# PacificBiosciences/trgt

Hardware: AMD Instinct MI355X
Metric: loci/s (higher is better)
Workload: dtype u8/u16 (WFA) + f64 (HMM); 1 GPU; BASELINE configs[1]: 10000 synthetic single-motif STR loci per GPU (motif 3-6 bp, allele <= 200 bp), 30 reads/locus HiFi-like, 10% truncated reads (SURVEY.md Appendix E), seed 20250509; contexts_per_gpu=4, loci_per_gpu=10000, reads_per_locus=30, parallelism=loci sharded across 1 GPU(s), no collective

## Files before the change

trgt_amd/csrc/common.hpp:

```cpp
#pragma once
#include <hip/hip_runtime.h>

#include <cstdarg>
#include <cstdint>
#include <cstdio>
#include <cstring>
#include <ctime>
#include <algorithm>
#include <mutex>
#include <string>
#include <vector>

#include "../../include/trgt_hip.h"

#ifdef TRGT_DEV_BUILD
#define TRGT_DEV_ENV(name) getenv(name)
#else
#define TRGT_DEV_ENV(name) ((const char*)nullptr)
#endif

struct trgt_knobs {
  int filter_force = 0;
  int flank_threads = 256;
  int heavy_band = 96;
// ... 16 lines not shown
  bool no_indel_shortcut = false;
  bool no_hamming = false;
  bool no_filter = false;
  bool one_stream = false;
  bool host_genotyper = false;
  bool no_early = false;
  bool stage_lock = false;
  bool host_hmm_lists = false;
  bool debug = false;
  bool hmm_resolve_one_wg = false;
  bool wfa_no_wave_variant = false;
  bool wfa_no_stage = false;
  bool filter_side = false;
  bool filter_serial = false;
  bool filter_one_launch = false;
  bool no_long_window = false;
  bool no_long_filter = false;
  bool no_lean = false;
  bool lean_mid_tier = false;
  int lean_chunk = 0;
  bool no_zero_arena = false;
  bool hmm_ppl_per_class = false;
  bool hmm_ppl_wide = false;
  bool hmm_ppl_serial = false;
  bool lean_one_tier = false;
  bool no_lds_wfa = true;
  int lds_wfa_kb = 7;
  int lds_wfa_seq = 768;
  int sens_bialign_min_len = -1;
  bool sens_cons_unidir = false;
  bool sens_ward_ties = false;
  bool sens_lw_order = false;
  bool hmm_no_dedupe = false;
  bool hmm_no_long_tb = false;
  int hmm_long_wgs = 4;
  bool hmm_no_ppl = false;
  bool hmm_four_rounds = false;
  bool hmm_lds_fill = false;
  int cluster_arena_kb = 0;
  int repair_arena_kb = 0;
  bool host_cluster = false;
  bool host_purity = false;
  bool host_repair = false;
  bool split_hmm = false;
  int repair_blocks = 2048;
  int repair_max_seg = 0;
// ... 491 lines not shown
```

trgt_amd/csrc/ctx.hip:

```cpp
#include "common.hpp"
#include "host_pool.hpp"

static std::string g_create_err;

#include <malloc.h>
static void tune_malloc_once() {
  static std::once_flag once;
  std::call_once(once, [] {
    const char* e = getenv("TRGT_MALLOC_TUNE");
    const int mode = e && *e ? atoi(e) : 1;
    if (mode <= 0) return;
    (void)mallopt(M_MMAP_THRESHOLD, 32 << 20);
    (void)mallopt(M_TRIM_THRESHOLD, 1 << 30);
    (void)mallopt(M_TOP_PAD, 64 << 20);
    if (mode >= 2) (void)mallopt(M_MMAP_MAX, 0);
  });
}

namespace trgt {
static thread_local int g_next_stream_priority = 0;
static thread_local bool g_next_in_pool = false;
void ctx_next_stream_priority(int p) { g_next_stream_priority = p; }
void ctx_next_in_pool(bool on) { g_next_in_pool = on; }
hipError_t make_stream(trgt_hip_ctx* c, hipStream_t* s) {
// ... 34 lines not shown
    return TRGT_ERR_NO_DEVICE;
  }
  tune_malloc_once();
  trgt_hip_ctx* c = new trgt_hip_ctx();
  {
    trgt_knobs& k = c->knobs;
    auto num = [](const char* name, int dflt) { const char* e = getenv(name); return e && *e ? atoi(e) : dflt; };
    auto flag = [](const char* name) { const char* e = getenv(name); return e != nullptr && *e != 0 && std::strcmp(e, "0") != 0; };
#ifdef TRGT_DEV_BUILD
#define DEV_FLAG(name) flag(name)
#define DEV_NUM(name, dflt) num(name, dflt)
#else
#define DEV_FLAG(name) false
#define DEV_NUM(name, dflt) (dflt)
#endif
    (void)num; (void)flag;
    k.flank_threads = DEV_NUM("TRGT_FLANK_THREADS", k.flank_threads); k.heavy_threads = DEV_NUM("TRGT_HEAVY_THREADS", 0); k.heavy_band = std::max(0, std::min(num("TRGT_HEAVY_BAND", k.heavy_band), 256));
    k.win_threads = DEV_NUM("TRGT_WIN_THREADS", k.win_threads); { const int bt = DEV_NUM("TRGT_BAND_THREADS", k.band_threads); k.band_threads = bt == 128 || bt == 256 ? bt : 64; } k.win_segments = DEV_NUM("TRGT_WIN_SEGMENTS", k.win_segments); k.win_lds = DEV_FLAG("TRGT_WIN_LDS"); k.band_lds = DEV_FLAG("TRGT_BAND_LDS");
    k.grid_per_cu = DEV_NUM("TRGT_WFA_GRID_PER_CU", 0); k.filter_per_cu = DEV_NUM("TRGT_FILTER_PER_CU", 0);
    k.one_launch = DEV_FLAG("TRGT_WFA_ONE_LAUNCH"); k.no_spec = DEV_FLAG("TRGT_WFA_NO_SPEC"); k.no_window = flag("TRGT_WFA_NO_WINDOW"); k.no_hamming = flag("TRGT_NO_HAMMING"); k.no_indel_shortcut = flag("TRGT_NO_INDEL_SHORTCUT"); k.no_heavy_window = DEV_FLAG("TRGT_NO_HEAVY_WINDOW"); k.no_sibling_rule = DEV_FLAG("TRGT_NO_SIBLING_RULE"); k.no_settled_sibling_rule = DEV_FLAG("TRGT_NO_SETTLED_SIBLING_RULE"); k.no_lcs_rule = DEV_FLAG("TRGT_NO_LCS_RULE"); { const char* e = TRGT_DEV_ENV("TRGT_EARLY_ADAPTIVE"); if (e && *e) k.early_adaptive = std::strcmp(e, "0") != 0; }
    k.no_filter = flag("TRGT_WFA_NO_FILTER"); k.one_stream = DEV_FLAG("TRGT_FLANK_ONE_STREAM"); k.host_genotyper = flag("TRGT_HOST_GENOTYPER"); k.host_hmm_lists = DEV_FLAG("TRGT_HOST_HMM_LISTS"); k.no_early = flag("TRGT_WFA_NO_EARLY"); k.stage_lock = flag("TRGT_STAGE_LOCK"); k.no_long_filter = flag("TRGT_NO_LONG_FILTER"); k.no_long_window = DEV_FLAG("TRGT_NO_LONG_WINDOW"); k.filter_force = DEV_NUM("TRGT_FILTER_FORCE", 0); k.filter_one_launch = DEV_FLAG("TRGT_FILTER_ONE_LAUNCH"); k.filter_serial = DEV_FLAG("TRGT_FILTER_SERIAL"); k.filter_side = DEV_FLAG("TRGT_FILTER_SIDE"); k.wfa_no_stage = DEV_FLAG("TRGT_WFA_NO_STAGE"); k.wfa_no_wave_variant = DEV_FLAG("TRGT_WFA_NO_WAVE_VARIANT"); k.hmm_resolve_one_wg = DEV_FLAG("TRGT_HMM_RESOLVE_ONE_WG"); k.debug = flag("TRGT_WFA_DEBUG");
    k.timeline = flag("TRGT_TIMELINE");
    k.host_repair = flag("TRGT_HOST_REPAIR"); k.host_cluster = flag("TRGT_HOST_CLUSTER"); k.host_purity = DEV_FLAG("TRGT_HOST_PURITY"); k.cluster_arena_kb = num("TRGT_CLUSTER_ARENA_KB", 0); k.repair_arena_kb = num("TRGT_REPAIR_ARENA_KB", 0); k.hmm_lds_fill = DEV_FLAG("TRGT_HMM_LDS_FILL"); k.hmm_four_rounds = DEV_FLAG("TRGT_HMM_FOUR_ROUNDS"); k.hmm_no_ppl = flag("TRGT_HMM_NO_PPL"); k.hmm_long_wgs = std::max(1, std::min(DEV_NUM("TRGT_HMM_LONG_WGS", k.hmm_long_wgs), 16)); k.hmm_no_long_tb = flag("TRGT_HMM_NO_LONG_TB"); k.hmm_no_dedupe = flag("TRGT_HMM_NO_DEDUPE"); k.repair_max_seg = num("TRGT_REPAIR_MAX_SEG", k.repair_max_seg); k.split_hmm = DEV_FLAG("TRGT_SPLIT_HMM"); k.repair_blocks = DEV_NUM("TRGT_REPAIR_BLOCKS", k.repair_blocks);
    k.no_lean = flag("TRGT_WFA_NO_LEAN"); k.lean_one_tier = DEV_FLAG("TRGT_WFA_LEAN_ONE_TIER"); k.lean_mid_tier = DEV_FLAG("TRGT_WFA_LEAN_MID_TIER"); k.lean_chunk = DEV_NUM("TRGT_LEAN_CHUNK", 0); k.no_zero_arena = flag("TRGT_NO_ZERO_ARENA"); k.hmm_ppl_serial = DEV_FLAG("TRGT_HMM_PPL_SERIAL"); k.hmm_ppl_wide = DEV_FLAG("TRGT_HMM_PPL_WIDE"); k.hmm_ppl_per_class = DEV_FLAG("TRGT_HMM_PPL_PER_CLASS");
    k.no_lds_wfa = !DEV_FLAG("TRGT_WFA_LDS"); k.lds_wfa_kb = DEV_NUM("TRGT_WFA_LDS_KB", k.lds_wfa_kb); k.lds_wfa_seq = DEV_NUM("TRGT_WFA_LDS_SEQ", k.lds_wfa_seq);
#ifdef TRGT_DEV_BUILD
    k.sens_bialign_min_len = num("TRGT_SENS_BIALIGN_MIN_LEN", -1); k.sens_cons_unidir = flag("TRGT_SENS_CONS_UNIDIR"); k.sens_ward_ties = flag("TRGT_SENS_WARD_TIES"); k.sens_lw_order = flag("TRGT_SENS_LW_ORDER");
    k.skip_bt = flag("TRGT_DBG_SKIP_BT");
#endif
  }
  c->device = device;
  c->num_cus = prop.multiProcessorCount;
  c->stream_priority = trgt::g_next_stream_priority;
  c->in_pool = trgt::g_next_in_pool;
  e = trgt::make_stream(c, &c->stream);
  if (e != hipSuccess) { g_create_err = hipGetErrorString(e); delete c; return TRGT_ERR_HIP; }
  c->own_stream = true;
  c->pool.resize(trgt::S_COUNT);
  *out = c;
  return TRGT_OK;
}

void trgt_hip_destroy(trgt_hip_ctx* c) {
  if (!c) return;
  (void)hipSetDevice(c->device);
  (void)trgt::stream_wait(c, c->stream);
  if (c->stream2) { (void)trgt::stream_wait(c, c->stream2); (void)hipStreamDestroy(c->stream2); }
// ... 92 lines not shown
```

trgt_amd/csrc/hmm.hip:

```cpp
#include <algorithm>
#include <type_traits>
#include <cmath>
#include <limits>
#include <thread>

#include "common.hpp"

namespace trgt {


}
#include <memory>

#include "hmm_host.hpp"
namespace trgt {

struct HmmJobDev {
  uint32_t set, seq_len, job_index, path_cap;
  uint64_t seq_off, bp_off, path_off, span_off, count_off, visit_off;
  uint64_t map_off;
};

static inline uint64_t align_up(uint64_t v, uint64_t a) { return (v + a - 1) / a * a; }

// ... 433 lines not shown
  for (int i = tid; i < 4 * S; i += nthr) l_inst[4 * (i % S) + i / S] = hmm_pred_entry(g_inst[i], S, nb, model + set.off_flags, g_block, g_blocks);
  const bool own_fill = !(ppl_filled && set.ppl_lanes != 0u);
  for (int i = tid; i < S; i += nthr) { l_block[i] = g_block[i]; l_flags[i] = model[set.off_flags + i]; if (own_fill) { l_lp[i] = g_inlp[i]; l_lp[S + i] = g_inlp[S + i]; } }
  if (own_fill) for (int i = tid; i < 5 * S; i += nthr) l_em[i] = g_em[i];
  for (int i = tid; i < 4 * nb; i += nthr) l_blocks[i] = g_blocks[i];

  const int st_lane = set.n_lanes ? (int)reinterpret_cast<const uint16_t*>(model + set.off_perm)[tid] : tid;
  const bool act = st_lane < S;
  const int st = act ? st_lane : 0;
  const int n_in = own_fill ? (int)model[set.off_nin + st] : 0;
  const int level = own_fill ? (int)model[set.off_level + st] : 0;
  double lp0 = 0.0, lp1 = 0.0, lp2 = 0.0, lp3 = 0.0;
  int p0 = 0, p1 = 0, p2 = 0, p3 = 0;
  if (own_fill) {
    lp0 = g_inlp[0 * S + st]; lp1 = g_inlp[1 * S + st]; lp2 = g_inlp[2 * S + st]; lp3 = g_inlp[3 * S + st];
    p0 = g_inst[0 * S + st]; p1 = g_inst[1 * S + st]; p2 = g_inst[2 * S + st]; p3 = g_inst[3 * S + st];
  }
  const int q0 = (n_in != 0xFF && n_in > 0) ? p0 : 0, q1 = (n_in != 0xFF && n_in > 1) ? p1 : 0, q2 = (n_in != 0xFF && n_in > 2) ? p2 : 0, q3 = (n_in != 0xFF && n_in > 3) ? p3 : 0;
  const uint8_t* __restrict__ seq = seq_blob + job.seq_off;
  int win0 = 0;
  auto code_at = [&](int i) -> int { return (int)l_seq[i - win0]; };
  uint8_t* __restrict__ bp = bp_ws + job.bp_off;
  hmm_sync_mem(sync_n);
  if (act) {
    const int blk = (int)l_block[st];
    uint32_t kind = 0, expected = 0;
    if (blk >= 0) {
      const int bstart = (int)l_blocks[0 * nb + blk], bend = (int)l_blocks[1 * nb + blk];
      if (st == bstart) kind = 1;
      else if (st == bend) kind = 2;
      else if (blk == nb - 1) kind = 3;
      else {
        const int mlen = (int)l_blocks[2 * nb + blk], off = st - bstart - 1, k = off / mlen;
        kind = 4u + (uint32_t)k;
        if (k == 0) expected = motif_bytes[l_blocks[3 * nb + blk] + off];
      }
    }
    l_info[st] = kind | ((uint32_t)(l_flags[st] & 1) << 3) | ((uint32_t)(blk & 0xFF) << 8) | (expected << 16);
  }
  const int my_blk = act ? (int)l_block[st] : -1;
  const bool role_end = act && my_blk >= 0 && st == (int)l_blocks[1 * nb + my_blk];
  const bool role_start = act && my_blk >= 0 && st == (int)l_blocks[0 * nb + my_blk];
  const bool role_del = act && level > 0 && !role_end && !role_start && n_in != 0xFF && my_blk >= 0;
  const bool role_chain = role_del || role_end;
  const bool chain_prev = role_del ? n_in > 1 : role_end ? n_in > 2 : false;
  const bool chain_xwave = chain_prev && (threadIdx.x & 63u) == 0;
  const double lp_chain = role_del ? lp1 : lp2, lp_step = chain_prev && !chain_xwave ? lp_chain : NINF;
  const int chain_steps = __builtin_amdgcn_readfirstlane(min(63, max((int)set.max_mlen, SUB == 32 ? __shfl_xor((int)set.max_mlen, 32) : 0) - 1));
  const int chain_rounds = (int)set.chain_rounds;
  const bool wave_chain = __ballot(lp_step > NINF) != 0ull;

  HP_MARK(0);
  const double lp_rs0 = l_lp[1], lp_rs1 = l_lp[S + 1];
  constexpr int BE_REG = 8;
  int be[BE_REG];
#pragma unroll
  for (int b = 0; b < BE_REG; ++b) be[b] = (int)l_blocks[1 * nb + (b < nb ? b : 0)];
  const int my_ms = my_blk >= 0 ? (int)l_blocks[0 * nb + my_blk] : 0, my_me = my_blk >= 0 ? (int)l_blocks[1 * nb + my_blk] : 0;
  const double ms_lp0 = my_blk >= 0 ? l_lp[my_ms] : NINF, ms_lp1 = my_blk >= 0 ? l_lp[S + my_ms] : NINF;
  bool bad = false, use_loc0 = false, use_loc1 = false;
  if (own_fill && act && my_blk >= 0) bad = model[set.off_nin + my_ms] != 2 || g_inst[0 * S + my_ms] != 1 || g_inst[1 * S + my_ms] != my_me;
  if (own_fill && act && level == 0 && n_in != 0xFF) {
// ... 449 lines not shown
  hmm_sync_mem(sync_n);

  const bool packed = ppl_filled && ppl_packed && set.ppl_lanes != 0u;
  const int rstride = packed ? hmm_ppl_group(set.ppl_lanes) : Spad;
  const int cols_per_chunk = packed ? hmm_stage_bytes(Spad) / rstride - 2 : max(1, hmm_stage_bytes(Spad) / Spad);
  if (tid == 0) tb[TB_LOC] = 0;
  uint16_t* pbuf = path ? path + job.path_off : nullptr;
  uint32_t* const g_vis = visit_ws + job.visit_off;
  const int pcap = (int)job.path_cap;
  constexpr int HMM_REC = SUB == 32 ? 32 : 64;
  const unsigned long long gmask = SUB == 32 ? (0xFFFFFFFFull << (threadIdx.x & 32u)) : ~0ull;
  const HmmSyncN sync{sync_n};
  const HmmTraceLds tl{tb, l_inst, l_info, l_blocks, l_flags, l_stage, l_seq, l_mot, l_vis, l_cnt, l_rec};
  hmm_trace_rounds<HMM_REC, true>(sync, tid, nthr, tl, packed, rstride, cols_per_chunk, S, nb, L, seq, bp, g_vis, pbuf, pcap, gmask);
  const int np = tb[TB_NPATH];
  HP_MARK(2);
  hmm_path_to_front(sync, tid, nthr, pbuf, np, pcap);
  if (tid == 0) hmm_store_purity(job.job_index, np, tb[TB_EDIT], tb[TB_REF], qlen, path_len, purity, edit_out, maxd_out);
  hmm_decode_visits(sync, tid, nthr, tl, nb, g_vis, spans3 + 3 * job.span_off, n_spans + job.job_index, counts + job.count_off);
  HP_MARK(3);
}

#include "hmm_ppl.hpp"
#include "hmm_big.hpp"

struct HmmChunkMap { uint16_t exit_state, last_state, n_steps, n_starts; int32_t last_end; };
struct HmmChunkRec { uint32_t entry, np0, nv0; int32_t vb0, nxt0; uint32_t pad[3]; };
constexpr int HMM_LONG_THREADS = 1024, HMM_LONG_STG = 2048;
constexpr int HMM_LONG_MAP_LDS = 48 * 1024;

__global__ void __launch_bounds__(HMM_LONG_THREADS) hmm_traceback_long_kernel(
    const HmmJobDev* __restrict__ jobs, const HmmSetDev* __restrict__ sets, const uint8_t* __restrict__ model, const uint8_t* __restrict__ seq_blob,
    const uint8_t* __restrict__ bp_ws, uint32_t* __restrict__ visit_ws, uint16_t* __restrict__ path, uint32_t* __restrict__ path_len,
    int32_t* __restrict__ spans3, uint32_t* __restrict__ n_spans, uint32_t* __restrict__ counts, double* __restrict__ purity,
    int32_t* __restrict__ edit_out, int32_t* __restrict__ maxd_out, const uint32_t* __restrict__ long_list, const int phase_arg, const int G) {
  const int phase = phase_arg & 0xFF;
  const bool ppl_packed = ((phase_arg >> 8) & 1) != 0;
  extern __shared__ __align__(16) unsigned char lds_long[];
  const int tid = (int)threadIdx.x, lane = tid & 63, wave = tid >> 6;
  constexpr int NW = HMM_LONG_THREADS / 64;
  const int part = (int)(blockIdx.x % (unsigned)G);
  __shared__ int l_last;
  for (uint32_t li = blockIdx.x / (unsigned)G; li < long_list[0]; li += gridDim.x / (unsigned)G) {
    __syncthreads();
    const HmmJobDev job = jobs[long_list[1 + li]];
    const HmmSetDev set = sets[job.set];
// ... 499 lines not shown
```

trgt_amd/csrc/hmm_batch.hpp:

```cpp
#pragma once

static inline uint32_t hmm_long_min(uint64_t class_jobs) { return class_jobs <= 256 ? 512u : (uint32_t)HMM_LONG_MIN; }
static inline uint64_t hmm_map_words(uint32_t S, uint64_t max_len, uint32_t long_min) {
  const uint64_t L = max_len + 2;
  if (L < (uint64_t)long_min) return 0;
  const uint64_t n_chunks = (L + HMM_LONG_CHUNK - 1) / HMM_LONG_CHUNK;
  return n_chunks * (3ull * S + 8ull) + 8;
}
static size_t hmm_long_lds_bytes(uint32_t S, uint32_t nb) {
  size_t o = 64 + (size_t)20 * S + (size_t)20 * nb + ((S + 3) & ~3u) + (((size_t)S / 3 + 15) & ~(size_t)15) + 32;
  return ((o + 15) & ~(size_t)15) + (size_t)(HMM_LONG_THREADS / 64) * (HMM_LONG_STG + 512) + HMM_LONG_MAP_LDS;
}
static size_t hmm_lds_bytes(uint32_t S, uint32_t nb) {
  size_t o = 64 + (((size_t)HMM_LDS_PER_STATE * S + 15) & ~(size_t)15) + (((size_t)16 * nb + 15) & ~(size_t)15) + (size_t)hmm_stage_bytes((int)((S + 15) & ~15u));
  o += HMM_CODE_WINDOW + HMM_CODE_PAD + (((size_t)S / 3 + 15) & ~(size_t)15) + 12 * (size_t)HMM_VIS_LDS + 4 * (size_t)nb;
  o += 8 + 8 * 64;
  return o + 64;
}


constexpr uint32_t HMM_BATCH_MAX_WAVES = 16, HMM_SLOT_MAX_WAVES = 7, HMM_CLASS_BIG = 17;
static inline uint32_t hmm_set_class(const HmmSetDev& sd, uint32_t max_waves) {
  if (sd.S <= 32) return 0u;
  const uint32_t w = (std::max(sd.S, sd.n_lanes) + 63) / 64;
// ... 70 lines not shown
  bool ppl_launched;
  size_t first_job, n_listed;
  int64_t cells;
  unsigned* side_used;
  HmmLaunchBufs b;
};
constexpr size_t HMM_LONG_PIECE_PAD = 16;

static uint32_t hmm_viterbi_flags(const trgt_hip_ctx* c, size_t lds_job, unsigned ppl_mask, uint32_t long_min) {
  return (uint32_t)lds_job | (c->knobs.hmm_four_rounds ? 0x80000000u : 0u) | (ppl_mask ? 0x40000000u : 0u) | (ppl_mask && !c->knobs.hmm_ppl_wide ? 0x00800000u : 0u) | ((long_min / 256u) << 24);
}
struct HmmViterbiFn {
  const void* fn;
  void (*launch)(dim3 grid, dim3 block, size_t lds, hipStream_t ls, const HmmClassLaunch& a, uint32_t flags, uint32_t* d_long);
};
template <int SUB, bool ONE_WAVE>
static void hmm_launch_viterbi(dim3 grid, dim3 block, size_t lds, hipStream_t ls, const HmmClassLaunch& a, uint32_t flags, uint32_t* d_long) {
  hipLaunchKernelGGL((hmm_viterbi_kernel<SUB, ONE_WAVE>), grid, block, lds, ls, a.jobs, a.b.sets, a.b.model, a.b.seq, a.b.bp, a.b.visits, a.b.path, a.b.plen, a.b.spans,
                     a.b.nsp, a.b.cnt, a.b.pur, a.b.edit, a.b.maxd, a.nj, flags, a.n_jobs_dev, d_long);
}
template <int SUB, bool ONE_WAVE>
static HmmViterbiFn hmm_viterbi_fn() { return {(const void*)hmm_viterbi_kernel<SUB, ONE_WAVE>, hmm_launch_viterbi<SUB, ONE_WAVE>}; }

static int hmm_fork_record(trgt_hip_ctx* c, int buffer_set) {
  hipEvent_t& ev = c->hmm_fork[buffer_set ? 1 : 0];
  if (!ev) TRGT_HIP_TRY(c, hipEventCreateWithFlags(&ev, hipEventDisableTiming));
  TRGT_HIP_TRY(c, hipEventRecord(ev, c->stream));
  return TRGT_OK;
}
static int hmm_class_stream(trgt_hip_ctx* c, int buffer_set, int ordinal, unsigned& side_used, hipStream_t* ls) {
  *ls = c->stream;
  if (ordinal == 0) return TRGT_OK;
  const int sidx = (ordinal - 1) % 3 + (buffer_set ? 3 : 0);
  if (!c->hmm_side[sidx]) TRGT_HIP_TRY(c, make_side_stream(c, &c->hmm_side[sidx]));
  if (!c->hmm_join[sidx]) TRGT_HIP_TRY(c, hipEventCreateWithFlags(&c->hmm_join[sidx], hipEventDisableTiming));
  *ls = c->hmm_side[sidx];
  TRGT_HIP_TRY(c, hipStreamWaitEvent(*ls, c->hmm_fork[buffer_set ? 1 : 0], 0));
  side_used |= 1u << sidx;
  return TRGT_OK;
}
static int hmm_join_classes(trgt_hip_ctx* c, unsigned side_used) {
  for (int sidx = 0; sidx < 6; ++sidx)
    if (side_used & (1u << sidx)) {
      TRGT_HIP_TRY(c, hipEventRecord(c->hmm_join[sidx], c->hmm_side[sidx]));
      TRGT_HIP_TRY(c, hipStreamWaitEvent(c->stream, c->hmm_join[sidx], 0));
    }
// ... 14 lines not shown
  hipStream_t ls;
  if ((rc = hmm_class_stream(c, a.buffer_set, a.ordinal, *a.side_used, &ls))) return rc;
  KTimer t(c, TRGT_K_HMM, ls);
  const HmmLaunchBufs& b = a.b;
  if (big) {
    if ((rc = hmm_launch_big(c, ls, a.maxS, a.maxnb, a.nj, a.jobs, b.sets, b.model, b.seq, b.bp, b.visits, b.path, b.plen, b.spans, b.nsp, b.cnt, b.pur, b.edit, b.maxd, a.n_jobs_dev))) return rc;
    t.stop(a.cells);
    return TRGT_OK;
  }
  uint32_t* d_long_cls = nullptr;
  const uint32_t long_min_cls = hmm_long_min(a.nj);
  if (!c->knobs.hmm_no_long_tb && a.max_len + 2 >= (uint64_t)long_min_cls) {
    if (void* z = zero_take(c, ((size_t)a.nj + 16) * 4)) d_long_cls = (uint32_t*)z;
    else {
      void* dl = nullptr;
      const int so = a.buffer_set ? (int)S_HMM_B_BASE - (int)S_HMM_SEQ : 0;
      if ((rc = dev_get(c, S_HMM_LONG + so, (a.n_listed + HMM_LONG_PIECE_PAD * (HMM_CLASS_BIG + 1)) * 4, &dl))) return rc;
      d_long_cls = (uint32_t*)dl + a.first_job + HMM_LONG_PIECE_PAD * (size_t)a.ordinal;
      TRGT_HIP_TRY(c, hipMemsetAsync(d_long_cls, 0, 4, ls));
    }
  }
  if (a.ppl_mask && !a.ppl_launched &&
      (rc = hmm_launch_ppl(c, a.buffer_set ? 1 : 0, a.ordinal & 3, ls, a.ppl_mask, a.jobs, b.sets, b.model, b.seq, b.bp, hmm_ppl_one_segment(a.nj, a.n_jobs_dev)))) return rc;
  k.launch(dim3(half ? (a.nj + 1) / 2 : a.nj), dim3(half ? 64 : 64 * a.cls), lds, ls, a, hmm_viterbi_flags(c, lds_job, a.ppl_mask, long_min_cls), d_long_cls);
  TRGT_HIP_TRY(c, hipGetLastError());
  if (d_long_cls) {
    const size_t llds = hmm_long_lds_bytes(a.maxS, a.maxnb);
    if (llds > 64 * 1024) TRGT_HIP_TRY(c, hipFuncSetAttribute((const void*)hmm_traceback_long_kernel, hipFuncAttributeMaxDynamicSharedMemorySize, (int)llds));
    const int G = c->knobs.hmm_long_wgs;
    for (int ph = G > 1 ? 1 : 0; ph <= (G > 1 ? 3 : 0); ++ph) {
      const int g = ph == 1 || ph == 3 ? G : 1;
      hipLaunchKernelGGL(hmm_traceback_long_kernel, dim3((unsigned)std::min<uint32_t>(a.nj, 64u) * (unsigned)g), dim3(HMM_LONG_THREADS), llds, ls, a.jobs, b.sets, b.model, b.seq,
                         (const uint8_t*)b.bp, b.visits, b.path, b.plen, b.spans, b.nsp, b.cnt, b.pur, b.edit, b.maxd, (const uint32_t*)d_long_cls,
                         ph | (a.ppl_mask && !c->knobs.hmm_ppl_wide ? 0x100 : 0), g);
    }
    TRGT_HIP_TRY(c, hipGetLastError());
  }
  t.stop(a.cells);
  return TRGT_OK;
}

int hmm_build_models(int32_t n_sets, const uint8_t* motif_blob, const uint32_t* motif_off, const uint32_t* set_motif_begin, HmmModels& out) {
  char msg[160];
  out.rc = 0;
  std::vector<HmmSetDev>& sets = out.sets;
  sets.assign((size_t)n_sets, HmmSetDev());
  std::vector<std::vector<uint8_t>> blobs((size_t)n_sets);
// ... 658 lines not shown
```

trgt_amd/csrc/hmm_traceback.hpp:

```cpp
#pragma once

struct HmmSyncN {
  int n;
  __device__ __forceinline__ void lds() const { hmm_sync(n); }
  __device__ __forceinline__ void mem() const { hmm_sync_mem(n); }
};
struct HmmSyncBlock {
  __device__ __forceinline__ void lds() const { asm volatile("s_waitcnt lgkmcnt(0)\n\ts_barrier" ::: "memory"); }
  __device__ __forceinline__ void mem() const { __syncthreads(); }
};

struct HmmStepCarry { int np, nv, nxt, vb; };
struct HmmStepSums { int edit, ref, n_starts, last_state, idx_last_end; bool any_end; };

template <int REC, class CodeAt, class VisAt>
__device__ __forceinline__ HmmStepSums hmm_decode_steps(const int slot, const int n, const HmmStepCarry cy, const unsigned long long gmask,
                                                        const uint32_t* l_rec, const uint32_t* l_info, const uint32_t* l_blocks, const int nb,
                                                        const uint8_t* motif_bytes, uint16_t* pbuf, const int pcap, CodeAt code_at, VisAt vis_at) {
  const int hwlane = (int)(threadIdx.x & 63u);
  const unsigned long long below = gmask & ((1ull << hwlane) - 1ull);
  const bool valid = slot < n;
  const int state = valid ? (int)l_rec[2 * slot] : 0, idx = valid ? (int)l_rec[2 * slot + 1] : 0;
  const uint32_t inf = valid ? l_info[state] : 0u;
  const int kind = (int)(inf & 7u), blk = (int)((inf >> 8) & 0xFFu), expected = (int)((inf >> 16) & 0xFFu);
// ... 41 lines not shown
__device__ __forceinline__ void hmm_path_to_front(const Sync sync, const int tid, const int nthr, uint16_t* pbuf, const int np, const int pcap) {
  if (!pbuf) return;
  const int n = min(np, pcap), shift = pcap - n;
  sync.mem();
  for (int base = 0; base < n; base += nthr) {
    const int f = base + tid;
    uint16_t v = 0;
    if (f < n) v = pbuf[shift + f];
    sync.mem();
    if (f < n) pbuf[f] = v;
    sync.mem();
  }
}

__device__ __forceinline__ void hmm_store_purity(const uint32_t job_index, const int np, const int edit, const int ref, const int qlen, uint32_t* path_len,
                                                 double* purity, int32_t* edit_out, int32_t* maxd_out) {
  if (path_len) path_len[job_index] = (uint32_t)np;
  const int mx = max(ref, qlen);
  purity[job_index] = ((double)mx - (double)edit) / (double)mx;
  if (edit_out) edit_out[job_index] = edit;
  if (maxd_out) maxd_out[job_index] = mx;
}

struct HmmTraceLds {
  int* tb;
  const uint32_t* inst;
  const uint32_t* info;
  const uint32_t* blocks;
  const uint8_t* flags;
  uint8_t* stage;
  uint8_t* seq;
  const uint8_t* mot;
  uint32_t* vis;
  uint32_t* cnt;
  uint32_t* rec;
};
enum { TB_STATE = 0, TB_IDX, TB_DONE, TB_NPATH, TB_NVISIT, TB_EDIT, TB_REF, TB_NEXT, TB_VB1,
       TB_NREC,
       TB_MORE,
       TB_LOC };
__device__ __forceinline__ void hmm_trace_init(int* tb, const int S, const int L) {
  tb[TB_STATE] = S - 1; tb[TB_IDX] = L - 1; tb[TB_DONE] = 0; tb[TB_NPATH] = 0; tb[TB_NVISIT] = 0; tb[TB_EDIT] = 0; tb[TB_REF] = 0; tb[TB_NEXT] = -1; tb[TB_VB1] = 0;
}

template <int REC, bool PPL, class Sync>
__device__ __forceinline__ void hmm_trace_rounds(const Sync sync, const int tid, const int nthr, const HmmTraceLds l, const bool packed_arg, const int rstride,
                                                 const int cols_per_chunk, const int S, const int nb, const int L, const uint8_t* __restrict__ seq,
                                                 const uint8_t* bp, uint32_t* g_vis, uint16_t* pbuf, const int pcap, const unsigned long long gmask) {
  const bool packed = PPL && packed_arg;
  int* const tb = l.tb;
  while (true) {
    if (tb[TB_DONE]) break;
    const int c1 = tb[TB_IDX] + 1, c0 = packed ? (max(0, c1 - cols_per_chunk) & ~1) : max(0, c1 - cols_per_chunk);
    {
      const uint4* src = reinterpret_cast<const uint4*>(bp + (size_t)c0 * rstride);
      uint4* dst = reinterpret_cast<uint4*>(l.stage);
      const int n16 = ((c1 - c0) * rstride + 15) / 16;
      for (int i = tid; i < n16; i += nthr) dst[i] = src[i];
      for (int k = tid; k < c1 - c0 + HMM_CODE_PAD && c0 + k < L; k += nthr) l.seq[k] = (uint8_t)hmm_code(seq, c0 + k, L);
    }
    auto code_at = [&](int i) -> int { return (int)l.seq[i - c0]; };
    sync.lds();
    for (;;) {
      if (tid == 0) {
        int state = tb[TB_STATE], idx = tb[TB_IDX], n = 0;
        int row = (idx - c0) * rstride;
        int emits = (int)((l.info[state] >> 3) & 1u);
        uint32_t loc = PPL ? (uint32_t)tb[TB_LOC] : 0u;
        while (state != 0 && idx >= c0 && n < REC) {
          l.rec[2 * n] = (uint32_t)state; l.rec[2 * n + 1] = (uint32_t)idx; ++n;
          const uint4 pred4 = *reinterpret_cast<const uint4*>(l.inst + 4 * state);
          int b;
          if (packed) {
            b = (int)hmm_bp_unpack(l.stage[row + (int)(loc & 63u)], loc);
            if (state == S - 2) b = (int)hmm_bp_run_end(*reinterpret_cast<const uint32_t*>(l.stage + row));
          } else b = l.stage[row + state];
          uint32_t pe = (b & 2) ? ((b & 1) ? pred4.w : pred4.z) : ((b & 1) ? pred4.y : pred4.x);
          if (state == S - 2) {
            const int bb = PPL ? b : (b < nb ? b : 0);
            const uint32_t be_ = l.blocks[1 * nb + bb];
            pe = be_ | ((uint32_t)(l.flags[be_] & 1) << 15);
            if (PPL) pe |= hmm_bp_loc_block_end(bb, nb, l.blocks) << 16;
          }
          if (emits) { --idx; row -= rstride; }
          emits = (int)((pe >> 15) & 1u);
          state = (int)(pe & 0x7FFFu);
          loc = pe >> 16;
        }
        tb[TB_STATE] = state; tb[TB_IDX] = idx; tb[TB_NREC] = n;
        if (PPL) tb[TB_LOC] = (int)loc;
        tb[TB_MORE] = state == 0 ? 2 : (idx >= c0 ? 1 : 0);
      }
      sync.lds();
      const int more = tb[TB_MORE];
      if (tid < REC) {
        const int n = tb[TB_NREC];
        const HmmStepCarry cy{tb[TB_NPATH], tb[TB_NVISIT], tb[TB_NEXT], tb[TB_VB1]};
        const HmmStepSums r = hmm_decode_steps<REC>(tid, n, cy, gmask, l.rec, l.info, l.blocks, nb, l.mot, pbuf, pcap, code_at,
                                                    [&](int nv) -> uint32_t* { return nv < HMM_VIS_LDS ? l.vis + 3 * nv : g_vis + 3 * (size_t)nv; });
        if (tid == 0) {
          int np = cy.np + n;
          if (more == 2) { if (pbuf && np < pcap) pbuf[pcap - 1 - np] = 0; ++np; tb[TB_DONE] = 1; }
          tb[TB_NPATH] = np; tb[TB_NVISIT] = cy.nv + r.n_starts; tb[TB_EDIT] += r.edit; tb[TB_REF] += r.ref;
          if (n > 0) tb[TB_NEXT] = r.last_state;
          if (r.any_end) tb[TB_VB1] = r.idx_last_end;
        }
      }
      sync.lds();
      if (more != 1) break;
    }
  }
}

template <class Sync>
__device__ __forceinline__ void hmm_decode_visits(const Sync sync, const int tid, const int nthr, const HmmTraceLds l, const int nb, const uint32_t* g_vis,
                                                  int32_t* const sp, uint32_t* n_spans_job, uint32_t* counts_job) {
  const int n_motifs = nb - 1;
  int ns = 0, cum = 0, last_motif = -1, last_end = -1;
  auto take_visit = [&](const uint32_t* vrec) {
    const int blk = (int)(vrec[0] & 0x7FFFu), b0 = (int)vrec[1], b1 = (int)vrec[2];
    const bool keep = (vrec[0] >> 15) == 0;
    const int cnt = b1 - b0;
    const int start = cum, end = cum + cnt;
    cum = end;
    const int motif = keep ? blk : nb - 1;
    if (motif < n_motifs) {
      l.cnt[motif] += 1;
      if (ns > 0 && last_motif == motif && last_end == start) { sp[3 * (ns - 1) + 2] = end; }
      else { sp[3 * ns + 0] = motif; sp[3 * ns + 1] = start; sp[3 * ns + 2] = end; ++ns; last_motif = motif; }
      last_end = end;
    }
  };
  int v = l.tb[TB_NVISIT] - 1;
  constexpr int VIS_CHUNK = HMM_STAGE_BYTES / 12;
  uint32_t* const l_vchunk = reinterpret_cast<uint32_t*>(l.stage);
  while (v >= HMM_VIS_LDS) {
    const int n = min(v - HMM_VIS_LDS + 1, VIS_CHUNK), v0 = v - n + 1;
    sync.mem();
    for (int k = tid; k < 3 * n; k += nthr) l_vchunk[k] = g_vis[3 * (size_t)v0 + k];
    sync.lds();
    if (tid == 0) for (int k = n - 1; k >= 0; --k) take_visit(l_vchunk + 3 * k);
    v -= n;
  }
  if (tid == 0) {
    for (; v >= 0; --v) take_visit(l.vis + 3 * v);
    *n_spans_job = (uint32_t)ns;
  }
  sync.lds();
  for (int m = tid; m < n_motifs; m += nthr) counts_job[m] = l.cnt[m];
}
```

Before: 4.932 million loci/s.

## Pack HMM traceback jobs into 8/16-lane groups per wavefront for small models

Adds a dedicated traceback kernel that runs several HMM jobs per 64-lane wavefront (8 or 16 lanes each) for class-0 pipelined jobs with small state and block counts. Each job gets its own LDS slice, and a compile-time chunked staging path loads backpointers and symbol codes into registers before writing them to LDS. The aim is to stop wasting most of a wavefront on tiny traceback jobs and to raise occupancy. In exchange it adds a new code path with tighter LDS visit buffers, which means more spills to global memory for long paths, and it duplicates the model setup.

```diff
diff --git a/trgt_amd/csrc/common.hpp b/trgt_amd/csrc/common.hpp
--- a/trgt_amd/csrc/common.hpp
+++ b/trgt_amd/csrc/common.hpp
@@ -62,6 +62,7 @@
   bool no_zero_arena = false;
   bool hmm_ppl_per_class = false;
   bool hmm_ppl_wide = false;
+  bool hmm_trace_wide = false;
   bool hmm_ppl_serial = false;
   bool lean_one_tier = false;
   bool no_lds_wfa = true;
diff --git a/trgt_amd/csrc/ctx.hip b/trgt_amd/csrc/ctx.hip
--- a/trgt_amd/csrc/ctx.hip
+++ b/trgt_amd/csrc/ctx.hip
@@ -80,7 +80,7 @@
     k.no_filter = flag("TRGT_WFA_NO_FILTER"); k.one_stream = DEV_FLAG("TRGT_FLANK_ONE_STREAM"); k.host_genotyper = flag("TRGT_HOST_GENOTYPER"); k.host_hmm_lists = DEV_FLAG("TRGT_HOST_HMM_LISTS"); k.no_early = flag("TRGT_WFA_NO_EARLY"); k.stage_lock = flag("TRGT_STAGE_LOCK"); k.no_long_filter = flag("TRGT_NO_LONG_FILTER"); k.no_long_window = DEV_FLAG("TRGT_NO_LONG_WINDOW"); k.filter_force = DEV_NUM("TRGT_FILTER_FORCE", 0); k.filter_one_launch = DEV_FLAG("TRGT_FILTER_ONE_LAUNCH"); k.filter_serial = DEV_FLAG("TRGT_FILTER_SERIAL"); k.filter_side = DEV_FLAG("TRGT_FILTER_SIDE"); k.wfa_no_stage = DEV_FLAG("TRGT_WFA_NO_STAGE"); k.wfa_no_wave_variant = DEV_FLAG("TRGT_WFA_NO_WAVE_VARIANT"); k.hmm_resolve_one_wg = DEV_FLAG("TRGT_HMM_RESOLVE_ONE_WG"); k.debug = flag("TRGT_WFA_DEBUG");
     k.timeline = flag("TRGT_TIMELINE");
     k.host_repair = flag("TRGT_HOST_REPAIR"); k.host_cluster = flag("TRGT_HOST_CLUSTER"); k.host_purity = DEV_FLAG("TRGT_HOST_PURITY"); k.cluster_arena_kb = num("TRGT_CLUSTER_ARENA_KB", 0); k.repair_arena_kb = num("TRGT_REPAIR_ARENA_KB", 0); k.hmm_lds_fill = DEV_FLAG("TRGT_HMM_LDS_FILL"); k.hmm_four_rounds = DEV_FLAG("TRGT_HMM_FOUR_ROUNDS"); k.hmm_no_ppl = flag("TRGT_HMM_NO_PPL"); k.hmm_long_wgs = std::max(1, std::min(DEV_NUM("TRGT_HMM_LONG_WGS", k.hmm_long_wgs), 16)); k.hmm_no_long_tb = flag("TRGT_HMM_NO_LONG_TB"); k.hmm_no_dedupe = flag("TRGT_HMM_NO_DEDUPE"); k.repair_max_seg = num("TRGT_REPAIR_MAX_SEG", k.repair_max_seg); k.split_hmm = DEV_FLAG("TRGT_SPLIT_HMM"); k.repair_blocks = DEV_NUM("TRGT_REPAIR_BLOCKS", k.repair_blocks);
-    k.no_lean = flag("TRGT_WFA_NO_LEAN"); k.lean_one_tier = DEV_FLAG("TRGT_WFA_LEAN_ONE_TIER"); k.lean_mid_tier = DEV_FLAG("TRGT_WFA_LEAN_MID_TIER"); k.lean_chunk = DEV_NUM("TRGT_LEAN_CHUNK", 0); k.no_zero_arena = flag("TRGT_NO_ZERO_ARENA"); k.hmm_ppl_serial = DEV_FLAG("TRGT_HMM_PPL_SERIAL"); k.hmm_ppl_wide = DEV_FLAG("TRGT_HMM_PPL_WIDE"); k.hmm_ppl_per_class = DEV_FLAG("TRGT_HMM_PPL_PER_CLASS");
+    k.no_lean = flag("TRGT_WFA_NO_LEAN"); k.lean_one_tier = DEV_FLAG("TRGT_WFA_LEAN_ONE_TIER"); k.lean_mid_tier = DEV_FLAG("TRGT_WFA_LEAN_MID_TIER"); k.lean_chunk = DEV_NUM("TRGT_LEAN_CHUNK", 0); k.no_zero_arena = flag("TRGT_NO_ZERO_ARENA"); k.hmm_ppl_serial = DEV_FLAG("TRGT_HMM_PPL_SERIAL"); k.hmm_ppl_wide = DEV_FLAG("TRGT_HMM_PPL_WIDE"); k.hmm_trace_wide = DEV_FLAG("TRGT_HMM_TRACE_WIDE"); k.hmm_ppl_per_class = DEV_FLAG("TRGT_HMM_PPL_PER_CLASS");
     k.no_lds_wfa = !DEV_FLAG("TRGT_WFA_LDS"); k.lds_wfa_kb = DEV_NUM("TRGT_WFA_LDS_KB", k.lds_wfa_kb); k.lds_wfa_seq = DEV_NUM("TRGT_WFA_LDS_SEQ", k.lds_wfa_seq);
 #ifdef TRGT_DEV_BUILD
     k.sens_bialign_min_len = num("TRGT_SENS_BIALIGN_MIN_LEN", -1); k.sens_cons_unidir = flag("TRGT_SENS_CONS_UNIDIR"); k.sens_ward_ties = flag("TRGT_SENS_WARD_TIES"); k.sens_lw_order = flag("TRGT_SENS_LW_ORDER");
diff --git a/trgt_amd/csrc/hmm.hip b/trgt_amd/csrc/hmm.hip
--- a/trgt_amd/csrc/hmm.hip
+++ b/trgt_amd/csrc/hmm.hip
@@ -479,22 +479,7 @@
   auto code_at = [&](int i) -> int { return (int)l_seq[i - win0]; };
   uint8_t* __restrict__ bp = bp_ws + job.bp_off;
   hmm_sync_mem(sync_n);
-  if (act) {
-    const int blk = (int)l_block[st];
-    uint32_t kind = 0, expected = 0;
-    if (blk >= 0) {
-      const int bstart = (int)l_blocks[0 * nb + blk], bend = (int)l_blocks[1 * nb + blk];
-      if (st == bstart) kind = 1;
-      else if (st == bend) kind = 2;
-      else if (blk == nb - 1) kind = 3;
-      else {
-        const int mlen = (int)l_blocks[2 * nb + blk], off = st - bstart - 1, k = off / mlen;
-        kind = 4u + (uint32_t)k;
-        if (k == 0) expected = motif_bytes[l_blocks[3 * nb + blk] + off];
-      }
-    }
-    l_info[st] = kind | ((uint32_t)(l_flags[st] & 1) << 3) | ((uint32_t)(blk & 0xFF) << 8) | (expected << 16);
-  }
+  if (act) l_info[st] = hmm_state_info(st, (int)l_block[st], nb, l_blocks, motif_bytes, l_flags[st]);
   const int my_blk = act ? (int)l_block[st] : -1;
   const bool role_end = act && my_blk >= 0 && st == (int)l_blocks[1 * nb + my_blk];
   const bool role_start = act && my_blk >= 0 && st == (int)l_blocks[0 * nb + my_blk];
@@ -990,6 +975,7 @@
 }
 
 #include "hmm_ppl.hpp"
+#include "hmm_trace_ppl.hpp"
 #include "hmm_big.hpp"
 
 struct HmmChunkMap { uint16_t exit_state, last_state, n_steps, n_starts; int32_t last_end; };
diff --git a/trgt_amd/csrc/hmm_batch.hpp b/trgt_amd/csrc/hmm_batch.hpp
--- a/trgt_amd/csrc/hmm_batch.hpp
+++ b/trgt_amd/csrc/hmm_batch.hpp
@@ -116,6 +116,24 @@
 template <int SUB, bool ONE_WAVE>
 static HmmViterbiFn hmm_viterbi_fn() { return {(const void*)hmm_viterbi_kernel<SUB, ONE_WAVE>, hmm_launch_viterbi<SUB, ONE_WAVE>}; }
 
+static inline bool hmm_trace_packed(const trgt_hip_ctx* c, const HmmClassLaunch& a) {
+  return a.cls == 0 && a.ppl_mask != 0 && (a.ppl_mask & ~3u) == 0 && !c->knobs.hmm_ppl_wide && !c->knobs.hmm_no_ppl && !c->knobs.hmm_trace_wide &&
+         a.maxS <= (uint32_t)HMM_TP_MAX_STATES && a.maxnb <= (uint32_t)HMM_TP_MAX_BLOCKS;
+}
+static void hmm_launch_trace_ppl(hipStream_t ls, const HmmClassLaunch& a, uint32_t long_min, uint32_t* d_long) {
+  HmmTracePplArgs t{a.jobs, a.b.sets, a.b.model, a.b.seq, (const uint8_t*)a.b.bp, a.b.visits, a.b.path, a.b.plen, a.b.spans, a.b.nsp, a.b.cnt, a.b.pur, a.b.edit, a.b.maxd,
+                    a.nj, a.n_jobs_dev, {0u, 0u}, (int)long_min, d_long, 0u};
+  t.lds_per_job[0] = (uint32_t)hmm_trace_ppl_lds(8, (int)a.maxS, (int)a.maxnb).total;
+  t.lds_per_job[1] = (uint32_t)hmm_trace_ppl_lds(16, (int)a.maxS, (int)a.maxnb).total;
+  const uint32_t blocks8 = (a.nj + 7) / 8, blocks16 = (a.nj + 3) / 4;
+  const size_t lds8 = 8 * (size_t)t.lds_per_job[0], lds16 = 4 * (size_t)t.lds_per_job[1];
+  if ((a.ppl_mask & 3u) == 3u) {
+    t.n_blocks8 = blocks8;
+    hipLaunchKernelGGL(hmm_trace_ppl_both_kernel, dim3(blocks8 + blocks16), dim3(64), std::max(lds8, lds16), ls, t);
+  } else if (a.ppl_mask & 1u) hipLaunchKernelGGL((hmm_trace_ppl_kernel<8>), dim3(blocks8), dim3(64), lds8, ls, t);
+  else hipLaunchKernelGGL((hmm_trace_ppl_kernel<16>), dim3(blocks16), dim3(64), lds16, ls, t);
+}
+
 static int hmm_fork_record(trgt_hip_ctx* c, int buffer_set) {
   hipEvent_t& ev = c->hmm_fork[buffer_set ? 1 : 0];
   if (!ev) TRGT_HIP_TRY(c, hipEventCreateWithFlags(&ev, hipEventDisableTiming));
@@ -176,7 +194,11 @@
   }
   if (a.ppl_mask && !a.ppl_launched &&
       (rc = hmm_launch_ppl(c, a.buffer_set ? 1 : 0, a.ordinal & 3, ls, a.ppl_mask, a.jobs, b.sets, b.model, b.seq, b.bp, hmm_ppl_one_segment(a.nj, a.n_jobs_dev)))) return rc;
-  k.launch(dim3(half ? (a.nj + 1) / 2 : a.nj), dim3(half ? 64 : 64 * a.cls), lds, ls, a, hmm_viterbi_flags(c, lds_job, a.ppl_mask, long_min_cls), d_long_cls);
+  const bool packed_trace = hmm_trace_packed(c, a);
+  if (c->knobs.debug) fprintf(stderr, "[hmm] class %u: %u jobs, trace-back by %s\n", a.cls, a.nj, packed_trace ? "hmm_trace_ppl_kernel" : "hmm_viterbi_kernel");
+  if (packed_trace) {
+    hmm_launch_trace_ppl(ls, a, long_min_cls, d_long_cls);
+  } else k.launch(dim3(half ? (a.nj + 1) / 2 : a.nj), dim3(half ? 64 : 64 * a.cls), lds, ls, a, hmm_viterbi_flags(c, lds_job, a.ppl_mask, long_min_cls), d_long_cls);
   TRGT_HIP_TRY(c, hipGetLastError());
   if (d_long_cls) {
     const size_t llds = hmm_long_lds_bytes(a.maxS, a.maxnb);
diff --git a/trgt_amd/csrc/hmm_trace_ppl.hpp b/trgt_amd/csrc/hmm_trace_ppl.hpp
--- /dev/null
+++ b/trgt_amd/csrc/hmm_trace_ppl.hpp
@@ -0,0 +1,141 @@
+#pragma once
+
+#include "hmm_trace_ppl_lds.hpp"
+static_assert(HMM_TP_CODE_PAD == HMM_CODE_PAD, "the window of symbol codes reaches as far behind the staged columns as hmm_trace_rounds fills it");
+static_assert(HMM_TP_COLS + 2 <= HMM_CODE_WINDOW, "a chunk's symbol codes fit the window");
+
+struct HmmTracePplArgs {
+  const HmmJobDev* jobs; const HmmSetDev* sets; const uint8_t* model; const uint8_t* seq_blob; const uint8_t* bp_ws; uint32_t* visit_ws;
+  uint16_t* path; uint32_t* path_len; int32_t* spans3; uint32_t* n_spans; uint32_t* counts; double* purity; int32_t* edit_out; int32_t* maxd_out;
+  uint32_t n_launch_jobs;
+  const uint32_t* n_jobs_dev;
+  uint32_t lds_per_job[2];
+  int long_min;
+  uint32_t* long_list;
+  uint32_t n_blocks8;
+};
+
+template <int G>
+__device__ __forceinline__ void hmm_trace_ppl_wave(const HmmTracePplArgs& a, const uint32_t block) {
+  const HmmJobDev* __restrict__ jobs = a.jobs; const HmmSetDev* __restrict__ sets = a.sets;
+  const uint8_t* __restrict__ model = a.model; const uint8_t* __restrict__ seq_blob = a.seq_blob; const uint8_t* __restrict__ bp_ws = a.bp_ws;
+  uint32_t* __restrict__ visit_ws = a.visit_ws; uint16_t* __restrict__ path = a.path; uint32_t* __restrict__ path_len = a.path_len;
+  int32_t* __restrict__ spans3 = a.spans3; uint32_t* __restrict__ n_spans = a.n_spans; uint32_t* __restrict__ counts = a.counts;
+  double* __restrict__ purity = a.purity; int32_t* __restrict__ edit_out = a.edit_out; int32_t* __restrict__ maxd_out = a.maxd_out;
+  uint32_t n_launch_jobs = a.n_launch_jobs;
+  const uint32_t* __restrict__ n_jobs_dev = a.n_jobs_dev; uint32_t* __restrict__ long_list = a.long_list;
+  const uint32_t lds_per_job = a.lds_per_job[G == 8 ? 0 : 1];
+  const int long_min = a.long_min;
+  static_assert(G == 8 || G == 16, "jobs of 8 or 16 lanes");
+  extern __shared__ __align__(16) unsigned char lds_all[];
+  constexpr int JPW = 64 / G;
+  if (n_jobs_dev) n_launch_jobs = *n_jobs_dev;
+  const int hw = (int)threadIdx.x, grp = hw / G, tid = hw % G;
+  const uint32_t jidx = block * (uint32_t)JPW + (uint32_t)grp;
+  bool live = jidx < n_launch_jobs;
+  HmmJobDev job{}; HmmSetDev set{};
+  set.S = 8; set.n_blocks = 1;
+  if (live) {
+    job = jobs[jidx];
+    set = sets[job.set];
+    live = hmm_ppl_group(set.ppl_lanes) == G;
+  }
+  const int S = (int)set.S, nb = (int)set.n_blocks, n_motifs = nb - 1;
+  const int qlen = (int)job.seq_len, L = qlen + 2;
+  if (live) {
+    for (int m = tid; m < n_motifs; m += G) counts[job.count_off + m] = 0;
+    if (qlen == 0) {
+      if (tid == 0) {
+        if (path_len) path_len[job.job_index] = 0;
+        n_spans[job.job_index] = 0;
+        purity[job.job_index] = __builtin_nan("");
+        if (edit_out) edit_out[job.job_index] = 0;
+        if (maxd_out) maxd_out[job.job_index] = 0;
+      }
+      live = false;
+    } else if (long_list && job.map_off && L >= long_min) {
+      if (tid == 0) long_list[1 + atomicAdd(long_list, 1u)] = jidx;
+      live = false;
+    }
+  }
+  if (live) {
+    unsigned char* const lds = lds_all + (size_t)grp * lds_per_job;
+    const HmmTracePplLds lay = hmm_trace_ppl_lds(G, S, nb);
+    int* const tb = reinterpret_cast<int*>(lds + lay.tb);
+    uint32_t* const l_inst = reinterpret_cast<uint32_t*>(lds + lay.inst);
+    uint32_t* const l_info = reinterpret_cast<uint32_t*>(lds + lay.info);
+    uint32_t* const l_blocks = reinterpret_cast<uint32_t*>(lds + lay.blocks);
+    uint8_t* const l_flags = lds + lay.flags;
+    uint8_t* const l_mot = lds + lay.mot;
+    uint32_t* const l_cnt = reinterpret_cast<uint32_t*>(lds + lay.cnt);
+    uint32_t* const l_rec = reinterpret_cast<uint32_t*>(lds + lay.rec);
+    uint32_t* const l_vis = reinterpret_cast<uint32_t*>(lds + lay.vis);
+    uint8_t* const l_seq = lds + lay.seq;
+    uint8_t* const l_stage = lds + lay.stage;
+    const uint16_t* g_inst = reinterpret_cast<const uint16_t*>(model + set.off_inst);
+    const int16_t* g_block = reinterpret_cast<const int16_t*>(model + set.off_block);
+    const uint32_t* g_blocks = reinterpret_cast<const uint32_t*>(model + set.off_blocks);
+    const uint8_t* g_flags = model + set.off_flags;
+    const uint8_t* g_motifs = model + set.off_motifs;
+    const int mot_bytes = (S - 7 - n_motifs) / 3;
+    const HmmSyncN sync{64};
+    constexpr int KS = HMM_TP_MAX_STATES / G, KB = 4 * HMM_TP_MAX_BLOCKS / G;
+    int16_t* const t_block = reinterpret_cast<int16_t*>(l_stage);
+    uint32_t r_inst[KS][4], r_blocks[KB];
+    int r_blk[KS];
+    uint32_t r_flag[KS];
+#pragma unroll
+    for (int k = 0; k < KS; ++k) {
+      const int st = tid + k * G;
+      const bool ok = st < S;
+#pragma unroll
+      for (int b = 0; b < 4; ++b) r_inst[k][b] = ok ? (uint32_t)g_inst[b * S + st] : 0u;
+      r_blk[k] = ok ? (int)g_block[st] : -1;
+      r_flag[k] = ok ? (uint32_t)g_flags[st] : 0u;
+    }
+#pragma unroll
+    for (int k = 0; k < KB; ++k) r_blocks[k] = tid + k * G < 4 * nb ? g_blocks[tid + k * G] : 0u;
+    const uint32_t r_mot = tid < mot_bytes ? (uint32_t)g_motifs[tid] : 0u;
+#pragma unroll
+    for (int k = 0; k < KS; ++k)
+      if (tid + k * G < S) { l_flags[tid + k * G] = (uint8_t)r_flag[k]; t_block[tid + k * G] = (int16_t)r_blk[k]; }
+#pragma unroll
+    for (int k = 0; k < KB; ++k) if (tid + k * G < 4 * nb) l_blocks[tid + k * G] = r_blocks[k];
+    if (tid < mot_bytes) l_mot[tid] = (uint8_t)r_mot;
+    for (int i = tid; i < n_motifs; i += G) l_cnt[i] = 0;
+    sync.lds();
+#pragma unroll
+    for (int k = 0; k < KS; ++k) {
+      const int st = tid + k * G;
+      if (st < S) {
+        uint4 pe;
+        pe.x = hmm_pred_entry(r_inst[k][0], S, nb, l_flags, t_block, l_blocks); pe.y = hmm_pred_entry(r_inst[k][1], S, nb, l_flags, t_block, l_blocks);
+        pe.z = hmm_pred_entry(r_inst[k][2], S, nb, l_flags, t_block, l_blocks); pe.w = hmm_pred_entry(r_inst[k][3], S, nb, l_flags, t_block, l_blocks);
+        *reinterpret_cast<uint4*>(l_inst + 4 * st) = pe;
+        l_info[st] = hmm_state_info(st, r_blk[k], nb, l_blocks, l_mot, r_flag[k]);
+      }
+    }
+    if (tid == 0) { hmm_trace_init(tb, S, L); tb[TB_LOC] = 0; }
+    sync.lds();
+    const uint8_t* const seq = seq_blob + job.seq_off;
+    const uint8_t* const bp = bp_ws + job.bp_off;
+    uint16_t* const pbuf = path ? path + job.path_off : nullptr;
+    uint32_t* const g_vis = visit_ws + job.visit_off;
+    const int pcap = (int)job.path_cap;
+    const unsigned long long gmask = ((1ull << G) - 1ull) << (grp * G);
+    const HmmTraceLds tl{tb, l_inst, l_info, l_blocks, l_flags, l_stage, l_seq, l_mot, l_vis, l_cnt, l_rec};
+    hmm_trace_rounds<G, true, HMM_TP_VIS, HMM_TP_COLS>(sync, tid, G, tl, true, G, HMM_TP_COLS, S, nb, L, seq, bp, g_vis, pbuf, pcap, gmask);
+    const int np = tb[TB_NPATH];
+    hmm_path_to_front(sync, tid, G, pbuf, np, pcap);
+    if (tid == 0) hmm_store_purity(job.job_index, np, tb[TB_EDIT], tb[TB_REF], qlen, path_len, purity, edit_out, maxd_out);
+    hmm_decode_visits<HMM_TP_VIS, hmm_trace_ppl_stage_bytes(G)>(sync, tid, G, tl, nb, g_vis, spans3 + 3 * job.span_off, n_spans + job.job_index, counts + job.count_off);
+  }
+}
+
+template <int G>
+__global__ void __launch_bounds__(64) hmm_trace_ppl_kernel(const HmmTracePplArgs a) { hmm_trace_ppl_wave<G>(a, blockIdx.x); }
+
+__global__ void __launch_bounds__(64) hmm_trace_ppl_both_kernel(const HmmTracePplArgs a) {
+  if (blockIdx.x < a.n_blocks8) hmm_trace_ppl_wave<8>(a, blockIdx.x);
+  else hmm_trace_ppl_wave<16>(a, blockIdx.x - a.n_blocks8);
+}
diff --git a/trgt_amd/csrc/hmm_trace_ppl_lds.hpp b/trgt_amd/csrc/hmm_trace_ppl_lds.hpp
--- /dev/null
+++ b/trgt_amd/csrc/hmm_trace_ppl_lds.hpp
@@ -0,0 +1,46 @@
+#pragma once
+
+#if defined(__HIPCC__) || defined(__CUDACC__)
+#define HMM_TP_HD __host__ __device__
+#else
+#define HMM_TP_HD
+#endif
+
+constexpr int HMM_TP_COLS = 64;
+constexpr int HMM_TP_VIS = 32;
+constexpr int HMM_TP_CODE_PAD = 16;
+constexpr int HMM_TP_MAX_STATES = 32, HMM_TP_MAX_BLOCKS = 8;
+
+struct HmmTracePplLds {
+  int tb;
+  int inst;
+  int info;
+  int blocks;
+  int flags;
+  int mot;
+  int cnt;
+  int rec;
+  int vis;
+  int seq;
+  int stage;
+  int total;
+};
+HMM_TP_HD constexpr int hmm_tp_up16(int v) { return (v + 15) & ~15; }
+HMM_TP_HD constexpr int hmm_trace_ppl_stage_bytes(int G) { return (HMM_TP_COLS + 2) * G; }
+HMM_TP_HD constexpr HmmTracePplLds hmm_trace_ppl_lds(int G, int S, int nb) {
+  HmmTracePplLds l{};
+  int o = 0;
+  l.tb = o; o += 64;
+  l.inst = o; o += 16 * S;
+  l.info = o; o += hmm_tp_up16(4 * S);
+  l.blocks = o; o += 16 * nb;
+  l.flags = o; o += hmm_tp_up16(S);
+  l.mot = o; o += hmm_tp_up16(S > 7 ? (S - 7) / 3 : 1);
+  l.cnt = o; o += hmm_tp_up16(4 * nb);
+  l.rec = o; o += 8 * G;
+  l.vis = o; o += 12 * HMM_TP_VIS;
+  l.seq = o; o += hmm_tp_up16(HMM_TP_COLS + 2 + HMM_TP_CODE_PAD);
+  l.stage = o; o += hmm_tp_up16(hmm_trace_ppl_stage_bytes(G));
+  l.total = o;
+  return l;
+}
diff --git a/trgt_amd/csrc/hmm_traceback.hpp b/trgt_amd/csrc/hmm_traceback.hpp
--- a/trgt_amd/csrc/hmm_traceback.hpp
+++ b/trgt_amd/csrc/hmm_traceback.hpp
@@ -87,6 +87,22 @@
   if (maxd_out) maxd_out[job_index] = mx;
 }
 
+__device__ __forceinline__ uint32_t hmm_state_info(const int st, const int blk, const int nb, const uint32_t* blocks, const uint8_t* motif_bytes, const uint32_t flags_st) {
+  uint32_t kind = 0, expected = 0;
+  if (blk >= 0) {
+    const int bstart = (int)blocks[0 * nb + blk], bend = (int)blocks[1 * nb + blk];
+    if (st == bstart) kind = 1;
+    else if (st == bend) kind = 2;
+    else if (blk == nb - 1) kind = 3;
+    else {
+      const int mlen = (int)blocks[2 * nb + blk], off = st - bstart - 1, k = off / mlen;
+      kind = 4u + (uint32_t)k;
+      if (k == 0) expected = motif_bytes[blocks[3 * nb + blk] + off];
+    }
+  }
+  return kind | ((flags_st & 1u) << 3) | ((uint32_t)(blk & 0xFF) << 8) | (expected << 16);
+}
+
 struct HmmTraceLds {
   int* tb;
   const uint32_t* inst;
@@ -108,7 +124,7 @@
   tb[TB_STATE] = S - 1; tb[TB_IDX] = L - 1; tb[TB_DONE] = 0; tb[TB_NPATH] = 0; tb[TB_NVISIT] = 0; tb[TB_EDIT] = 0; tb[TB_REF] = 0; tb[TB_NEXT] = -1; tb[TB_VB1] = 0;
 }
 
-template <int REC, bool PPL, class Sync>
+template <int REC, bool PPL, int VIS = HMM_VIS_LDS, int CHUNK = 0, class Sync>
 __device__ __forceinline__ void hmm_trace_rounds(const Sync sync, const int tid, const int nthr, const HmmTraceLds l, const bool packed_arg, const int rstride,
                                                  const int cols_per_chunk, const int S, const int nb, const int L, const uint8_t* __restrict__ seq,
                                                  const uint8_t* bp, uint32_t* g_vis, uint16_t* pbuf, const int pcap, const unsigned long long gmask) {
@@ -117,12 +133,27 @@
   while (true) {
     if (tb[TB_DONE]) break;
     const int c1 = tb[TB_IDX] + 1, c0 = packed ? (max(0, c1 - cols_per_chunk) & ~1) : max(0, c1 - cols_per_chunk);
-    {
+    if constexpr (CHUNK == 0) {
       const uint4* src = reinterpret_cast<const uint4*>(bp + (size_t)c0 * rstride);
       uint4* dst = reinterpret_cast<uint4*>(l.stage);
       const int n16 = ((c1 - c0) * rstride + 15) / 16;
       for (int i = tid; i < n16; i += nthr) dst[i] = src[i];
       for (int k = tid; k < c1 - c0 + HMM_CODE_PAD && c0 + k < L; k += nthr) l.seq[k] = (uint8_t)hmm_code(seq, c0 + k, L);
+    } else {
+      constexpr int U16 = (((CHUNK + 1) * REC + 15) / 16 + REC - 1) / REC, UC = (CHUNK + 1 + HMM_CODE_PAD + REC - 1) / REC;
+      const uint4* src = reinterpret_cast<const uint4*>(bp + (size_t)c0 * REC);
+      uint4* dst = reinterpret_cast<uint4*>(l.stage);
+      const int n16 = ((c1 - c0) * REC + 15) / 16, nc = min(c1 - c0 + HMM_CODE_PAD, L - c0);
+      uint4 r16[U16];
+      int rc[UC];
+#pragma unroll
+      for (int u = 0; u < U16; ++u) r16[u] = tid + u * REC < n16 ? src[tid + u * REC] : make_uint4(0u, 0u, 0u, 0u);
+#pragma unroll
+      for (int u = 0; u < UC; ++u) rc[u] = tid + u * REC < nc ? hmm_code(seq, c0 + tid + u * REC, L) : 0;
+#pragma unroll
+      for (int u = 0; u < U16; ++u) if (tid + u * REC < n16) dst[tid + u * REC] = r16[u];
+#pragma unroll
+      for (int u = 0; u < UC; ++u) if (tid + u * REC < nc) l.seq[tid + u * REC] = (uint8_t)rc[u];
     }
     auto code_at = [&](int i) -> int { return (int)l.seq[i - c0]; };
     sync.lds();
@@ -162,7 +193,7 @@
         const int n = tb[TB_NREC];
         const HmmStepCarry cy{tb[TB_NPATH], tb[TB_NVISIT], tb[TB_NEXT], tb[TB_VB1]};
         const HmmStepSums r = hmm_decode_steps<REC>(tid, n, cy, gmask, l.rec, l.info, l.blocks, nb, l.mot, pbuf, pcap, code_at,
-                                                    [&](int nv) -> uint32_t* { return nv < HMM_VIS_LDS ? l.vis + 3 * nv : g_vis + 3 * (size_t)nv; });
+                                                    [&](int nv) -> uint32_t* { return nv < VIS ? l.vis + 3 * nv : g_vis + 3 * (size_t)nv; });
         if (tid == 0) {
           int np = cy.np + n;
           if (more == 2) { if (pbuf && np < pcap) pbuf[pcap - 1 - np] = 0; ++np; tb[TB_DONE] = 1; }
@@ -177,7 +208,7 @@
   }
 }
 
-template <class Sync>
+template <int VIS = HMM_VIS_LDS, int STAGE = HMM_STAGE_BYTES, class Sync>
 __device__ __forceinline__ void hmm_decode_visits(const Sync sync, const int tid, const int nthr, const HmmTraceLds l, const int nb, const uint32_t* g_vis,
                                                   int32_t* const sp, uint32_t* n_spans_job, uint32_t* counts_job) {
   const int n_motifs = nb - 1;
@@ -197,10 +228,10 @@
     }
   };
   int v = l.tb[TB_NVISIT] - 1;
-  constexpr int VIS_CHUNK = HMM_STAGE_BYTES / 12;
+  constexpr int VIS_CHUNK = STAGE / 12;
   uint32_t* const l_vchunk = reinterpret_cast<uint32_t*>(l.stage);
-  while (v >= HMM_VIS_LDS) {
-    const int n = min(v - HMM_VIS_LDS + 1, VIS_CHUNK), v0 = v - n + 1;
+  while (v >= VIS) {
+    const int n = min(v - VIS + 1, VIS_CHUNK), v0 = v - n + 1;
     sync.mem();
     for (int k = tid; k < 3 * n; k += nthr) l_vchunk[k] = g_vis[3 * (size_t)v0 + k];
     sync.lds();
```

Result: faster. 5.138 million loci/s, median of 6 (+4.2%).
